# LIONS-EPFL/LEAF

Measured on NVIDIA B200. Metric: leaf_candidates_scored_per_sec, higher is better.
Workload: dtype bf16

## Files before the change

include/leaf_b200.h:

```cpp
#ifndef LEAF_B200_H_
#define LEAF_B200_H_

#include <stdint.h>

#ifdef __cplusplus
extern "C" {
#endif

typedef enum {
  LEAF_OK = 0,
  LEAF_ERR_INVALID = -1,
  LEAF_ERR_CUDA = -2,
  LEAF_ERR_STATE = -3,
  LEAF_ERR_UNSUPPORTED = -4
} leaf_status_t;

typedef struct leaf_engine* leaf_handle_t;

enum { LEAF_ACT_GELU_ERF = 0, LEAF_ACT_QUICK_GELU = 1 };
enum { LEAF_OBJ_L2 = 0, LEAF_OBJ_NEGL2 = 1, LEAF_OBJ_SIM = 2, LEAF_OBJ_DISSIM = 3 };
enum { LEAF_CTX = 77, LEAF_SOT = 49406, LEAF_EOT = 49407, LEAF_VOCAB = 49408, LEAF_N_MERGES = 48894 };
enum { LEAF_MAX_CAPTION_BYTES = 1000, LEAF_MAX_CAPTION_BYTES_LONG = 3560 };

typedef struct {
// ... 33 lines not shown

int leaf_load_bpe(leaf_handle_t h, const uint32_t* merge_pairs_host, int32_t n_merges);

int leaf_bind_weights(leaf_handle_t h, const leaf_weight_ptrs_t* w, void* stream);
int leaf_refresh_weights(leaf_handle_t h, void* stream);

int leaf_reserve(leaf_handle_t h, int32_t max_seqs);

int leaf_expand_tokenize(leaf_handle_t h, const uint8_t* caps, const int32_t* cap_off, int32_t B, int32_t n,
                         const int32_t* pos, const int32_t* chr, const int32_t* sel, const uint8_t* valid,
                         int32_t* tok_out, int32_t* len_out, int32_t* base_out, int32_t* status_out, void* stream);

int leaf_set_tokenizer_mode(leaf_handle_t h, int32_t mode);
int leaf_set_max_caption_bytes(leaf_handle_t h, int32_t bytes);

int leaf_load_words(leaf_handle_t h, const uint8_t* words_blob, const int32_t* words_off, int32_t n_words,
                    const uint8_t* abbrev_blob, const int32_t* abbrev_off, int32_t n_abbrev);
int leaf_constrain_mask(leaf_handle_t h, const uint8_t* caps, const int32_t* cap_off, int32_t B, int32_t n,
                        const int32_t* pos, const int32_t* chr, const int32_t* sel, uint8_t* valid_out,
                        int32_t* count_out, int32_t* status_out, void* stream);

int leaf_encode(leaf_handle_t h, const int32_t* tok, const int32_t* len, const int32_t* base, int32_t N,
                int32_t dedup_rows, int32_t dedup_group, int32_t trim_providers, int32_t normalize, float* feat_out, void* stream);

int leaf_score(leaf_handle_t h, const float* feat, const float* anchor, int32_t B, int32_t n, int32_t objective,
               float* loss_out, int32_t* best_out, float* best_feat_out, void* stream);

int leaf_topk(leaf_handle_t h, const float* score_a, const float* score_b, int32_t m, int32_t k, int32_t* idx_out,
              float* val_out, void* stream);

int leaf_train_reserve(leaf_handle_t h, int32_t max_seqs);
int leaf_forward_train(leaf_handle_t h, const int32_t* tok, const int32_t* len, int32_t N, float* feat_out,
                       int32_t rows_hint, int32_t max_len_hint, int64_t* generation_out, void* stream);
int leaf_backward(leaf_handle_t h, int64_t generation, const float* dfeat, int32_t dfeat_rows, const leaf_weight_ptrs_t* grads,
                  void* stream);

typedef void (*leaf_backward_hook_t)(int32_t layer, void* user);
int leaf_set_backward_hook(leaf_handle_t h, leaf_backward_hook_t fn, void* user);
int leaf_set_sm_budget(leaf_handle_t h, int32_t n_sms);

int leaf_adamw(leaf_handle_t h, float* params, const float* grads, float* exp_avg, float* exp_avg_sq, int64_t n,
               int64_t n_nodecay, float lr, float beta1, float beta2, float eps, float weight_decay, int32_t step,
               float grad_scale, void* stream);
int leaf_sumsq(leaf_handle_t h, const float* g, int64_t n, float* out, void* stream);
int leaf_scale(leaf_handle_t h, float* g, int64_t n, float s, void* stream);

int leaf_gemm_bf16(leaf_handle_t h, const void* A, const void* Bt, const float* bias, void* C,
                   int32_t M, int32_t N, int32_t K, int32_t epilogue, int32_t act, const int32_t* m_dev,
                   void* stream);
int leaf_gemm_bf16_mn(leaf_handle_t h, const void* A, const void* B, const float* bias, void* C, int32_t M, int32_t N,
                      int32_t K, int32_t epilogue, int32_t a_mn, void* stream);
int leaf_test_layernorm(leaf_handle_t h, const float* x, int32_t rows, const float* gamma, const float* beta, void* y,
                        void* stream);
int leaf_test_attention(leaf_handle_t h, const void* qkv, const int32_t* meta, int32_t N, void* out, void* stream);
int leaf_test_attention_bwd(leaf_handle_t h, const void* qkv, const void* o, const float* dout, const int32_t* meta, int32_t N,
                            int32_t T, void* dqkv, void* stream);
int leaf_set_prune_last(leaf_handle_t h, int32_t on);
int64_t leaf_launch_count(leaf_handle_t h, int32_t reset);
int64_t leaf_last_rows(leaf_handle_t h);
int leaf_set_timing(leaf_handle_t h, int32_t on);
double leaf_timing_ms(leaf_handle_t h, int32_t which, int32_t* launches);

#ifdef __cplusplus
}
#endif
#endif
```

leaf_b200/_native.py:

```python
import ctypes
import os

HERE = os.path.dirname(os.path.abspath(__file__))
LIB_PATH = os.environ.get("LEAF_B200_LIB") or os.path.join(HERE, "lib", "libleaf_b200.so")

c_int, c_void_p, c_float, c_i64 = ctypes.c_int32, ctypes.c_void_p, ctypes.c_float, ctypes.c_int64


class LeafCfg(ctypes.Structure):
    _fields_ = [("width", c_int), ("layers", c_int), ("heads", c_int), ("embed_dim", c_int), ("activation", c_int),
                ("ln_eps", c_float)]


class LeafLayerPtrs(ctypes.Structure):
    _fields_ = [(k, c_void_p) for k in (
        "ln1_w", "ln1_b", "in_proj_w", "in_proj_b", "q_w", "k_w", "v_w", "q_b", "k_b", "v_b", "out_w", "out_b",
        "ln2_w", "ln2_b", "fc1_w", "fc1_b", "fc2_w", "fc2_b")]


class LeafWeightPtrs(ctypes.Structure):
    _fields_ = [("token_embedding", c_void_p), ("positional_embedding", c_void_p), ("lnf_w", c_void_p),
                ("lnf_b", c_void_p), ("text_projection", c_void_p), ("projection_is_ew", c_int),
                ("layers", ctypes.POINTER(LeafLayerPtrs))]


SIGNATURES = {
    "leaf_create": (c_int, [ctypes.POINTER(LeafCfg), ctypes.POINTER(c_void_p)]),
    "leaf_destroy": (c_int, [c_void_p]),
    "leaf_last_error": (ctypes.c_char_p, []),
    "leaf_version": (ctypes.c_char_p, []),
    "leaf_load_bpe": (c_int, [c_void_p, c_void_p, c_int]),
    "leaf_bind_weights": (c_int, [c_void_p, ctypes.POINTER(LeafWeightPtrs), c_void_p]),
    "leaf_refresh_weights": (c_int, [c_void_p, c_void_p]),
    "leaf_reserve": (c_int, [c_void_p, c_int]),
    "leaf_expand_tokenize": (c_int, [c_void_p, c_void_p, c_void_p, c_int, c_int, c_void_p, c_void_p, c_void_p, c_void_p,
                                     c_void_p, c_void_p, c_void_p, c_void_p, c_void_p]),
    "leaf_set_tokenizer_mode": (c_int, [c_void_p, c_int]),
    "leaf_set_max_caption_bytes": (c_int, [c_void_p, c_int]),
    "leaf_load_words": (c_int, [c_void_p, c_void_p, c_void_p, c_int, c_void_p, c_void_p, c_int]),
    "leaf_constrain_mask": (c_int, [c_void_p, c_void_p, c_void_p, c_int, c_int, c_void_p, c_void_p, c_void_p, c_void_p, c_void_p,
                                    c_void_p, c_void_p]),
    "leaf_encode": (c_int, [c_void_p, c_void_p, c_void_p, c_void_p, c_int, c_int, c_int, c_int, c_int, c_void_p, c_void_p]),
    "leaf_score": (c_int, [c_void_p, c_void_p, c_void_p, c_int, c_int, c_int, c_void_p, c_void_p, c_void_p, c_void_p]),
    "leaf_topk": (c_int, [c_void_p, c_void_p, c_void_p, c_int, c_int, c_void_p, c_void_p, c_void_p]),
    "leaf_train_reserve": (c_int, [c_void_p, c_int]),
    "leaf_forward_train": (c_int, [c_void_p, c_void_p, c_void_p, c_int, c_void_p, c_int, c_int, ctypes.POINTER(c_i64), c_void_p]),
    "leaf_backward": (c_int, [c_void_p, c_i64, c_void_p, c_int, ctypes.POINTER(LeafWeightPtrs), c_void_p]),
    "leaf_set_backward_hook": (c_int, [c_void_p, c_void_p, c_void_p]),
    "leaf_set_sm_budget": (c_int, [c_void_p, c_int]),
    "leaf_adamw": (c_int, [c_void_p, c_void_p, c_void_p, c_void_p, c_void_p, c_i64, c_i64, ctypes.c_float, ctypes.c_float,
                           ctypes.c_float, ctypes.c_float, ctypes.c_float, c_int, ctypes.c_float, c_void_p]),
    "leaf_sumsq": (c_int, [c_void_p, c_void_p, c_i64, c_void_p, c_void_p]),
    "leaf_scale": (c_int, [c_void_p, c_void_p, c_i64, ctypes.c_float, c_void_p]),
    "leaf_gemm_bf16": (c_int, [c_void_p, c_void_p, c_void_p, c_void_p, c_void_p, c_int, c_int, c_int, c_int, c_int,
                               c_void_p, c_void_p]),
    "leaf_gemm_bf16_mn": (c_int, [c_void_p, c_void_p, c_void_p, c_void_p, c_void_p, c_int, c_int, c_int, c_int, c_int, c_void_p]),
    "leaf_test_layernorm": (c_int, [c_void_p, c_void_p, c_int, c_void_p, c_void_p, c_void_p, c_void_p]),
    "leaf_test_attention": (c_int, [c_void_p, c_void_p, c_void_p, c_int, c_void_p, c_void_p]),
    "leaf_test_attention_bwd": (c_int, [c_void_p, c_void_p, c_void_p, c_void_p, c_void_p, c_int, c_int, c_void_p, c_void_p]),
    "leaf_set_prune_last": (c_int, [c_void_p, c_int]),
    "leaf_launch_count": (c_i64, [c_void_p, c_int]),
    "leaf_last_rows": (c_i64, [c_void_p]),
    "leaf_set_timing": (c_int, [c_void_p, c_int]),
    "leaf_timing_ms": (ctypes.c_double, [c_void_p, c_int, ctypes.POINTER(c_int)]),
}

BACKWARD_HOOK = ctypes.CFUNCTYPE(None, c_int, c_void_p)

_lib = None


class LeafError(RuntimeError):
    pass


def lib():
    global _lib
    if _lib is None:
        if not os.path.exists(LIB_PATH):
            raise LeafError(f"{LIB_PATH} is missing: build it with `python -m leaf_b200.build` "
                            "(leaf_b200 has no CPU or PyTorch fallback)")
        L = ctypes.CDLL(LIB_PATH)
        for name, (res, args) in SIGNATURES.items():
            fn = getattr(L, name)
            fn.restype = res
            fn.argtypes = args
        _lib = L
    return _lib


def check(rc: int):
    if rc != 0:
        raise LeafError(f"leaf_b200 error {rc}: {lib().leaf_last_error().decode('utf-8', 'replace')}")
```

leaf_b200/csrc/engine.cu:

```cuda
#include <cuda.h>
#include <cuda_bf16.h>
#include <cuda_runtime.h>
#include <stdarg.h>
#include <stdint.h>
#include <stdio.h>
#include <stdlib.h>
#include <string.h>

#include <map>
#include <string>
#include <tuple>
#include <vector>

#include "../../include/leaf_b200.h"
#include "gemm2_sm100.cuh"
#include "gemm_sm100.cuh"
#include "k1_tables_host.h"
#include "constrain_kernel.cuh"
#include "k1_tokenize.cuh"
#include "tower_kernels.cuh"
#include "attention2.cuh"
#include "train_kernels.cuh"

using namespace leaf;
// ... 468 lines not shown
  CK(cudaGetLastError());
  return LEAF_OK;
}

template <typename... KArgs, typename... Args>
static cudaError_t launch_pdl(const leaf_engine* e, void (*kernel)(KArgs...), dim3 grid, dim3 block, cudaStream_t st, Args... args) {
  cudaLaunchConfig_t cfg{};
  cfg.gridDim = grid;
  cfg.blockDim = block;
  cfg.stream = st;
  cudaLaunchAttribute attr[1];
  attr[0].id = cudaLaunchAttributeProgrammaticStreamSerialization;
  attr[0].val.programmaticStreamSerializationAllowed = 1;
  cfg.attrs = attr;
  cfg.numAttrs = e->pdl ? 1 : 0;
  return cudaLaunchKernelEx(&cfg, kernel, static_cast<KArgs>(args)...);
}

static int launch_layernorm(leaf_engine* e, const float* x, const int* rows_dev, int rows_max, const int* gather,
                            const float* g, const float* b, __nv_bfloat16* y, cudaStream_t st,
                            const __nv_bfloat16* delta = nullptr, __nv_bfloat16* y_lo = nullptr) {
  const int W = e->cfg.width;
  const int vpl = W / 128;
  TimedSpan span(e, 1, st);
  long warps = rows_max;
  int blocks = static_cast<int>((warps + 7) / 8);
  const int cap = e->sm_count * 8;
  if (blocks > cap) blocks = cap;
  if (blocks < 1) blocks = 1;
#define LN_CASE(V) case V: CK(launch_pdl(e, layernorm_bf16_kernel<V>, dim3(blocks), dim3(256), st, x, rows_dev, rows_max, gather, W, g, b, e->cfg.ln_eps, y, delta, y_lo)); break;
  switch (vpl) {
    LN_CASE(1) LN_CASE(2) LN_CASE(3) LN_CASE(4) LN_CASE(5) LN_CASE(6) LN_CASE(7) LN_CASE(8)
    LN_CASE(9) LN_CASE(10) LN_CASE(11) LN_CASE(12) LN_CASE(13) LN_CASE(14) LN_CASE(15) LN_CASE(16)
    default: return fail(LEAF_ERR_INVALID, "unsupported width %d", W);
  }
#undef LN_CASE
  e->launches++;
  CK(cudaGetLastError());
  return LEAF_OK;
}

static int launch_attention(leaf_engine* e, const __nv_bfloat16* qkv, const int4* meta, int N, __nv_bfloat16* out, int last_only,
                            cudaStream_t st, long rows_cap_hint = 0) {
  if (rows_cap_hint <= 0) rows_cap_hint = static_cast<long>(N) * LEAF_CTX;
  const int H = e->cfg.heads, W = e->cfg.width;
  if (e->att_impl == 2 && static_cast<unsigned long long>(rows_cap_hint) * 3ull * W < (1ull << 32)) {
    const long ctas = (static_cast<long>(N) * H + AT2_WARPS - 1) / AT2_WARPS;
    const int grid2 = static_cast<int>(ctas < 2L * e->sm_count ? ctas : 2L * e->sm_count);
    attention2_kernel<<<grid2, AT2_WARPS * 32, AT2_SMEM_BYTES, st>>>(qkv, meta, N, H, W, out, last_only);
    e->launches++;
    CK(cudaGetLastError());
    return LEAF_OK;
  }
  const int grid = (N * H + ATT_WARPS - 1) / ATT_WARPS;
  CK(launch_pdl(e, attention_kernel, dim3(grid), dim3(ATT_WARPS * 32), st, qkv, meta, N, H, W, out, last_only));
  e->launches++;
  CK(cudaGetLastError());
  return LEAF_OK;
}

extern "C" int leaf_encode(leaf_handle_t e, const int32_t* tok, const int32_t* len, const int32_t* base, int32_t N,
                           int32_t dedup_rows, int32_t dedup_group, int32_t trim_providers, int32_t normalize, float* feat_out,
                           void* stream) {
  if (!e || !tok || !len || !feat_out) return fail(LEAF_ERR_INVALID, "null argument");
  if (!e->bound) return fail(LEAF_ERR_STATE, "weights not bound");
  if (N <= 0) return fail(LEAF_ERR_INVALID, "N=%d", N);
  if (N > e->max_seqs) return fail(LEAF_ERR_STATE, "workspace reserved for %d rows, need %d (leaf_reserve)", e->max_seqs, N);
  cudaStream_t st = static_cast<cudaStream_t>(stream);
  const int W = e->cfg.width, E = e->cfg.embed_dim;
  const int rows_max = static_cast<int>(static_cast<long>(N) * LEAF_CTX);
  int rc;
  const int* dup = nullptr;
  {
  TimedSpan span(e, 3, st);
  if (dedup_group > 1 && dedup_rows > 0) {
    if (dedup_rows > N || dedup_rows % dedup_group != 0) return fail(LEAF_ERR_INVALID, "dedup_rows=%d dedup_group=%d N=%d", dedup_rows, dedup_group, N);
    dedup_kernel<<<(N + 7) / 8, 256, 0, st>>>(tok, len, dedup_rows, dedup_group, N, e->dup_of);
    e->launches++;
    dup = e->dup_of;
  }
  const bool trim = trim_providers && base && dedup_rows > 0 && dedup_rows < N;
  if (trim) CK(cudaMemsetAsync(e->need, 0, static_cast<size_t>(N) * 4, st));
  prefix_kernel<<<(N + 7) / 8, 256, 0, st>>>(tok, len, base, dup, N, e->pfx, e->own_len, trim ? e->need : nullptr);
  if (trim) {
    trim_providers_kernel<<<(N - dedup_rows + 255) / 256, 256, 0, st>>>(base, e->need, dedup_rows, N, e->own_len);
    e->launches++;
  }
  scan_lengths_kernel<<<1, 1024, 0, st>>>(e->own_len, N, e->cu, e->total_rows);
  meta_kernel<<<(N + 255) / 256, 256, 0, st>>>(e->cu, e->pfx, base, dup, N, e->meta, e->eos_row, e->first_of);
  embed_kernel<<<N, 256, 0, st>>>(tok, e->meta, N, W, e->wp.token_embedding, e->wp.positional_embedding, e->x);
  e->launches += 4;
  }
  CK(cudaGetLastError());
  for (int l = 0; l < e->cfg.layers; ++l) {
    const leaf_layer_ptrs_t& p = e->layer_ptrs[l];
    const LayerW& w = e->lw[l];
    if ((rc = launch_layernorm(e, e->x, e->total_rows, rows_max, nullptr, p.ln1_w, p.ln1_b, e->h, st))) return rc;
    if ((rc = launch_gemm(e, e->h, e->rows_cap, w.qkv_w, w.qkv_b, e->big, 3 * W, rows_max, 3 * W, W, EPI_BF16, 0, e->total_rows, st))) return rc;
    const bool last = e->prune_last && l == e->cfg.layers - 1;
    const __nv_bfloat16* dl = e->dlt;
    {
      TimedSpan span(e, 2, st);
      if ((rc = launch_attention(e, e->big, e->meta, N, e->h, last ? 1 : 0, st))) return rc;
    }
    if (last) {
      {
        TimedSpan span(e, 3, st);
// ... 20 lines not shown
  if (normalize) {
    l2_normalize_kernel<<<(N + 7) / 8, 256, 0, st>>>(feat_out, N, E);
    e->launches++;
  }
  CK(cudaGetLastError());
  return LEAF_OK;
}

extern "C" int leaf_score(leaf_handle_t e, const float* feat, const float* anchor, int32_t B, int32_t n, int32_t objective,
                          float* loss_out, int32_t* best_out, float* best_feat_out, void* stream) {
  if (!e || !feat || !anchor || !best_out) return fail(LEAF_ERR_INVALID, "null argument");
  if (B <= 0 || n <= 0 || objective < 0 || objective > 3) return fail(LEAF_ERR_INVALID, "B=%d n=%d objective=%d", B, n, objective);
  if (e->cfg.embed_dim % 4 != 0) return fail(LEAF_ERR_INVALID, "embed_dim");
  if (static_cast<size_t>(n) * 4 > 48 * 1024) return fail(LEAF_ERR_INVALID, "n=%d too large", n);
  score_argmax_kernel<<<B, 256, static_cast<size_t>(n) * 4, static_cast<cudaStream_t>(stream)>>>(
      feat, anchor, n, e->cfg.embed_dim, objective, loss_out, best_out, best_feat_out);
  e->launches++;
  CK(cudaGetLastError());
  return LEAF_OK;
}

extern "C" int leaf_topk(leaf_handle_t e, const float* score_a, const float* score_b, int32_t m, int32_t k, int32_t* idx_out,
                         float* val_out, void* stream) {
  if (!e || !score_a || !idx_out) return fail(LEAF_ERR_INVALID, "null argument");
  if (m <= 0 || k <= 0 || k > m) return fail(LEAF_ERR_INVALID, "top-k of m=%d, k=%d", m, k);
  const size_t smem = static_cast<size_t>(m) * 4;
  if (smem > 200 * 1024) return fail(LEAF_ERR_INVALID, "m=%d too large (max %d)", m, 200 * 1024 / 4);
  topk_kernel<<<1, 1024, smem, static_cast<cudaStream_t>(stream)>>>(score_a, score_b, m, k, idx_out, val_out);
  e->launches++;
  CK(cudaGetLastError());
  return LEAF_OK;
}

extern "C" int leaf_gemm_bf16(leaf_handle_t e, const void* A, const void* Bt, const float* bias, void* C, int32_t M, int32_t N,
                              int32_t K, int32_t epilogue, int32_t act, const int32_t* m_dev, void* stream) {
  if (!e || !A || !Bt || !C) return fail(LEAF_ERR_INVALID, "null argument");
  return launch_gemm(e, static_cast<const __nv_bfloat16*>(A), M, static_cast<const __nv_bfloat16*>(Bt), bias, C, N, M, N, K,
                     epilogue, act, m_dev, static_cast<cudaStream_t>(stream));
}

extern "C" int leaf_gemm_bf16_mn(leaf_handle_t e, const void* A, const void* B, const float* bias, void* C, int32_t M, int32_t N,
                                 int32_t K, int32_t epilogue, int32_t a_mn, void* stream) {
  if (!e || !A || !B || !C) return fail(LEAF_ERR_INVALID, "null argument");
  return launch_gemm(e, static_cast<const __nv_bfloat16*>(A), a_mn ? K : M, static_cast<const __nv_bfloat16*>(B), bias, C, N, M, N, K,
                     epilogue, 0, nullptr, static_cast<cudaStream_t>(stream), nullptr, GEMM_B_MN | (a_mn ? GEMM_A_MN : 0));
}

extern "C" int leaf_test_layernorm(leaf_handle_t e, const float* x, int32_t rows, const float* gamma, const float* beta, void* y,
                                   void* stream) {
  if (!e || !x || !gamma || !beta || !y || rows <= 0) return fail(LEAF_ERR_INVALID, "bad argument");
  return launch_layernorm(e, x, nullptr, rows, nullptr, gamma, beta, static_cast<__nv_bfloat16*>(y), static_cast<cudaStream_t>(stream));
}

extern "C" int leaf_test_attention(leaf_handle_t e, const void* qkv, const int32_t* meta, int32_t N, void* out, void* stream) {
  if (!e || !qkv || !meta || !out || N <= 0) return fail(LEAF_ERR_INVALID, "bad argument");
  return launch_attention(e, static_cast<const __nv_bfloat16*>(qkv), reinterpret_cast<const int4*>(meta), N,
                          static_cast<__nv_bfloat16*>(out), 0, static_cast<cudaStream_t>(stream));
}

extern "C" int leaf_test_attention_bwd(leaf_handle_t e, const void* qkv, const void* o, const float* dout, const int32_t* meta,
                                       int32_t N, int32_t T, void* dqkv, void* stream) {
  if (!e || !qkv || !o || !dout || !meta || !dqkv || N <= 0 || T <= 0 || T > LEAF_CTX) return fail(LEAF_ERR_INVALID, "bad argument");
  attention_bwd_kernel<<<dim3(N, e->cfg.heads), ATTB_WARPS * 32, attb_smem_bytes(T), static_cast<cudaStream_t>(stream)>>>(
      static_cast<const __nv_bfloat16*>(qkv), static_cast<const __nv_bfloat16*>(o), dout, reinterpret_cast<const int4*>(meta),
      e->cfg.width, T, static_cast<__nv_bfloat16*>(dqkv));
  e->launches++;
  CK(cudaGetLastError());
  return LEAF_OK;
}

extern "C" int leaf_set_prune_last(leaf_handle_t e, int32_t on) {
  if (!e) return fail(LEAF_ERR_INVALID, "null handle");
  e->prune_last = on != 0;
  return LEAF_OK;
}

extern "C" int64_t leaf_launch_count(leaf_handle_t e, int32_t reset) {
  if (!e) return 0;
  const int64_t v = e->launches;
  if (reset) e->launches = 0;
  return v;
}

extern "C" int64_t leaf_last_rows(leaf_handle_t e) {
  if (!e || !e->total_rows) return 0;
  int v = 0;
  if (cudaMemcpy(&v, e->total_rows, 4, cudaMemcpyDeviceToHost) != cudaSuccess) return -1;
  return v;
}

extern "C" double leaf_timing_ms(leaf_handle_t e, int32_t which, int32_t* launches);
extern "C" int leaf_set_timing(leaf_handle_t e, int32_t on) {
  if (!e) return fail(LEAF_ERR_INVALID, "null handle");
  e->timing = on != 0;
  if (e->timing) {
    int32_t dummy;
    leaf_timing_ms(e, 0, &dummy);
    for (int i = 0; i < 10; ++i) { e->span_ms[i] = 0; e->span_n[i] = 0; }
  }
  return LEAF_OK;
}

extern "C" double leaf_timing_ms(leaf_handle_t e, int32_t which, int32_t* launches) {
  if (!e || which < 0 || which > 9) return 0.0;
  if (!e->spans.empty()) {
    for (auto& sp : e->spans) {
      cudaEventSynchronize(sp.b);
      float ms = 0.f;
      if (cudaEventElapsedTime(&ms, sp.a, sp.b) == cudaSuccess) {
        e->span_ms[sp.cat] += ms; e->span_n[sp.cat]++;
// ... 344 lines not shown
```

leaf_b200/csrc/tower_kernels.cuh:

```cuda
#pragma once
#include <cuda_bf16.h>
#include <cuda_runtime.h>
#include <stdint.h>

#include "gemm_sm100.cuh"

namespace leaf {

__device__ __forceinline__ float warp_sum(float v) {
#pragma unroll
  for (int o = 16; o > 0; o >>= 1) v += __shfl_xor_sync(0xffffffffu, v, o);
  return v;
}
__device__ __forceinline__ float warp_max(float v) {
#pragma unroll
  for (int o = 16; o > 0; o >>= 1) v = fmaxf(v, __shfl_xor_sync(0xffffffffu, v, o));
  return v;
}

__global__ void __launch_bounds__(1024) scan_lengths_kernel(const int* __restrict__ len, int N, int* __restrict__ cu,
                                                            int* __restrict__ total_rows, int* __restrict__ max_len = nullptr) {
  __shared__ int warp_tot[32];
  __shared__ int carry;
  __shared__ int vmax_s;
// ... 170 lines not shown
      pk.x = *reinterpret_cast<uint32_t*>(&lo);
      pk.y = *reinterpret_cast<uint32_t*>(&hi);
      out[lane + 32 * i] = pk;
      if (y_lo) {
        const float2 l = __bfloat1622float2(lo), h = __bfloat1622float2(hi);
        __nv_bfloat162 lo2 = __floats2bfloat162_rn((v[i].x - mean) * rstd * g.x + b.x - l.x, (v[i].y - mean) * rstd * g.y + b.y - l.y);
        __nv_bfloat162 hi2 = __floats2bfloat162_rn((v[i].z - mean) * rstd * g.z + b.z - h.x, (v[i].w - mean) * rstd * g.w + b.w - h.y);
        uint2 pk2;
        pk2.x = *reinterpret_cast<uint32_t*>(&lo2);
        pk2.y = *reinterpret_cast<uint32_t*>(&hi2);
        reinterpret_cast<uint2*>(y_lo + static_cast<size_t>(r) * W)[lane + 32 * i] = pk2;
      }
    }
  }
}

constexpr int ATT_WARPS = 4;

__device__ __forceinline__ void mma_bf16_16816(float* c, const uint32_t* a, uint32_t b0, uint32_t b1) {
  asm volatile(
      "mma.sync.aligned.m16n8k16.row.col.f32.bf16.bf16.f32 {%0,%1,%2,%3}, {%4,%5,%6,%7}, {%8,%9}, {%0,%1,%2,%3};"
      : "+f"(c[0]), "+f"(c[1]), "+f"(c[2]), "+f"(c[3])
      : "r"(a[0]), "r"(a[1]), "r"(a[2]), "r"(a[3]), "r"(b0), "r"(b1));
}
__device__ __forceinline__ uint32_t movmatrix_trans(uint32_t x) {
  uint32_t y;
  asm volatile("movmatrix.sync.aligned.m8n8.trans.b16 %0, %1;" : "=r"(y) : "r"(x));
  return y;
}
__device__ __forceinline__ uint32_t pack_bf16x2(float lo, float hi) {
  __nv_bfloat162 t = __floats2bfloat162_rn(lo, hi);
  return *reinterpret_cast<uint32_t*>(&t);
}
__device__ __forceinline__ float att_ex2(float x) {
  float y;
  asm("ex2.approx.ftz.f32 %0, %1;" : "=f"(y) : "f"(x));
  return y;
}

struct U8 { uint32_t r[8]; };
__device__ __forceinline__ U8 ldg256(const void* p) {
  U8 v;
  asm volatile("ld.global.nc.v8.b32 {%0,%1,%2,%3,%4,%5,%6,%7}, [%8];"
               : "=r"(v.r[0]), "=r"(v.r[1]), "=r"(v.r[2]), "=r"(v.r[3]), "=r"(v.r[4]), "=r"(v.r[5]), "=r"(v.r[6]), "=r"(v.r[7])
               : "l"(p));
  return v;
}
__device__ __forceinline__ void stg256(void* p, const U8& v) {
  asm volatile("st.global.v8.b32 [%0], {%1,%2,%3,%4,%5,%6,%7,%8};" ::"l"(p), "r"(v.r[0]), "r"(v.r[1]), "r"(v.r[2]), "r"(v.r[3]),
               "r"(v.r[4]), "r"(v.r[5]), "r"(v.r[6]), "r"(v.r[7])
               : "memory");
}

template <int NKT, int DEPTH>
__device__ __forceinline__ void attention_tile(const __nv_bfloat16* __restrict__ kbase, const __nv_bfloat16* __restrict__ vbase,
                                                  size_t ld, const U8& qa, const U8& qb, int pos0, int pos1, int t, int p,
                                                  int own_row, int base_row, int g, int c, float (&o)[8][4], float& inv0, float& inv1) {
  const float sl2 = 0.125f * 1.4426950408889634f;
  constexpr int NS = 2 * NKT;
  U8 ring[DEPTH][2];
  auto issue = [&](int si) {
    const int kt = si < NKT ? si : si - NKT;
    const __nv_bfloat16* src = si < NKT ? kbase : vbase;
#pragma unroll
    for (int h = 0; h < 2; ++h) {
      const int j = min(kt * 16 + h * 8 + g, t - 1);
      ring[si % DEPTH][h] = ldg256(src + static_cast<size_t>(j < p ? base_row + j : own_row + (j - p)) * ld);
    }
  };
#pragma unroll
  for (int si = 0; si < DEPTH && si < NS; ++si) issue(si);
  float s[NKT][2][4];
#pragma unroll
  for (int kt = 0; kt < NKT; ++kt) {
#pragma unroll
    for (int nt = 0; nt < 2; ++nt) {
      s[kt][nt][0] = s[kt][nt][1] = s[kt][nt][2] = s[kt][nt][3] = 0.f;
#pragma unroll
      for (int j = 0; j < 4; ++j) {
        const uint32_t a[4] = {qa.r[2 * j], qb.r[2 * j], qa.r[2 * j + 1], qb.r[2 * j + 1]};
        mma_bf16_16816(s[kt][nt], a, ring[kt % DEPTH][nt].r[2 * j], ring[kt % DEPTH][nt].r[2 * j + 1]);
      }
    }
    if (kt + DEPTH < NS) issue(kt + DEPTH);
  }
  float mx0 = -INFINITY, mx1 = -INFINITY;
#pragma unroll
  for (int kt = 0; kt < NKT; ++kt)
#pragma unroll
    for (int nt = 0; nt < 2; ++nt)
#pragma unroll
      for (int e = 0; e < 2; ++e) {
        const int j = kt * 16 + nt * 8 + 2 * c + e;
        if (j > pos0) s[kt][nt][e] = -INFINITY;
        if (j > pos1) s[kt][nt][2 + e] = -INFINITY;
        mx0 = fmaxf(mx0, s[kt][nt][e]);
        mx1 = fmaxf(mx1, s[kt][nt][2 + e]);
      }
  mx0 = fmaxf(mx0, __shfl_xor_sync(0xffffffffu, mx0, 1));
  mx0 = fmaxf(mx0, __shfl_xor_sync(0xffffffffu, mx0, 2));
  mx1 = fmaxf(mx1, __shfl_xor_sync(0xffffffffu, mx1, 1));
  mx1 = fmaxf(mx1, __shfl_xor_sync(0xffffffffu, mx1, 2));
  const float nm0 = -mx0 * sl2, nm1 = -mx1 * sl2;
  float l0 = 0.f, l1 = 0.f;
  uint32_t pf[NKT][4];
#pragma unroll
  for (int kt = 0; kt < NKT; ++kt)
#pragma unroll
    for (int nt = 0; nt < 2; ++nt) {
      const float p00 = att_ex2(fmaf(s[kt][nt][0], sl2, nm0)), p01 = att_ex2(fmaf(s[kt][nt][1], sl2, nm0));
      const float p10 = att_ex2(fmaf(s[kt][nt][2], sl2, nm1)), p11 = att_ex2(fmaf(s[kt][nt][3], sl2, nm1));
      l0 += p00 + p01;
      l1 += p10 + p11;
      pf[kt][2 * nt] = pack_bf16x2(p00, p01);
      pf[kt][2 * nt + 1] = pack_bf16x2(p10, p11);
    }
  l0 += __shfl_xor_sync(0xffffffffu, l0, 1);
  l0 += __shfl_xor_sync(0xffffffffu, l0, 2);
  l1 += __shfl_xor_sync(0xffffffffu, l1, 1);
  l1 += __shfl_xor_sync(0xffffffffu, l1, 2);
  inv0 = 1.f / l0;
  inv1 = 1.f / l1;
#pragma unroll
  for (int i = 0; i < 8; ++i) o[i][0] = o[i][1] = o[i][2] = o[i][3] = 0.f;
#pragma unroll
  for (int kt = 0; kt < NKT; ++kt) {
#pragma unroll
    for (int i = 0; i < 8; ++i)
      mma_bf16_16816(o[i], pf[kt], movmatrix_trans(ring[(NKT + kt) % DEPTH][0].r[i]), movmatrix_trans(ring[(NKT + kt) % DEPTH][1].r[i]));
    if (NKT + kt + DEPTH < NS) issue(NKT + kt + DEPTH);
  }
}

constexpr int ATT_DEPTH = 3;
__global__ void __launch_bounds__(ATT_WARPS * 32, 4) attention_kernel(const __nv_bfloat16* __restrict__ qkv,
                                                                       const int4* __restrict__ meta, int n_seq, int heads,
                                                                       int W, __nv_bfloat16* __restrict__ out,
                                                                       int last_only = 0) {
  pdl_wait();
  pdl_trigger();
  const int pair = blockIdx.x * ATT_WARPS + (threadIdx.x >> 5);
  if (pair >= n_seq * heads) return;
  const int seq = pair / heads, head = pair - seq * heads;
  const int lane = threadIdx.x & 31, g = lane >> 2, c = lane & 3;
  const int4 mt = __ldg(meta + seq);
  const int own_row = mt.x, t = mt.y, p = mt.z, base_row = mt.w;
  const int nq = t - p;
  if (nq <= 0) return;
  const size_t ld = static_cast<size_t>(3) * W;
  const __nv_bfloat16* qbase = qkv + head * 64 + c * 16;
  const __nv_bfloat16* kbase = qbase + W;
  const __nv_bfloat16* vbase = qbase + 2 * W;
  for (int q0 = last_only ? ((nq - 1) & ~15) : 0; q0 < nq; q0 += 16) {
    const int qi0 = min(q0 + g, nq - 1), qi1 = min(q0 + g + 8, nq - 1);
    const U8 qa = ldg256(qbase + static_cast<size_t>(own_row + qi0) * ld);
    const U8 qb = ldg256(qbase + static_cast<size_t>(own_row + qi1) * ld);
    const int pos0 = p + qi0, pos1 = p + qi1;
    const int kmax = min(t - 1, p + q0 + 15);
    float o[8][4];
    float inv0, inv1;
#define ATT_ARGS kbase, vbase, ld, qa, qb, pos0, pos1, t, p, own_row, base_row, g, c, o, inv0, inv1
    switch (kmax >> 4) {
      case 0: attention_tile<1, ATT_DEPTH>(ATT_ARGS); break;
      case 1: attention_tile<2, ATT_DEPTH>(ATT_ARGS); break;
      case 2: attention_tile<3, ATT_DEPTH>(ATT_ARGS); break;
      case 3: attention_tile<4, ATT_DEPTH>(ATT_ARGS); break;
      default: attention_tile<5, ATT_DEPTH>(ATT_ARGS); break;
    }
#undef ATT_ARGS
    U8 w0, w1;
#pragma unroll
    for (int i = 0; i < 8; ++i) {
      w0.r[i] = pack_bf16x2(o[i][0] * inv0, o[i][1] * inv0);
      w1.r[i] = pack_bf16x2(o[i][2] * inv1, o[i][3] * inv1);
    }
    __nv_bfloat16* ob = out + head * 64 + c * 16;
    if (last_only) {
      if (q0 + g == nq - 1) stg256(ob + static_cast<size_t>(seq) * W, w0);
      if (q0 + g + 8 == nq - 1) stg256(ob + static_cast<size_t>(seq) * W, w1);
    } else {
      if (q0 + g < nq) stg256(ob + static_cast<size_t>(own_row + q0 + g) * W, w0);
      if (q0 + g + 8 < nq) stg256(ob + static_cast<size_t>(own_row + q0 + g + 8) * W, w1);
    }
  }
}

__global__ void __launch_bounds__(256) gather_rows_f32_kernel(const float* __restrict__ src, const int* __restrict__ rows, int N,
                                                             int W, float* __restrict__ dst) {
  const int r = (blockIdx.x * blockDim.x + threadIdx.x) >> 5, lane = threadIdx.x & 31;
  if (r >= N) return;
  const float4* in = reinterpret_cast<const float4*>(src + static_cast<size_t>(rows[r]) * W);
  float4* o = reinterpret_cast<float4*>(dst + static_cast<size_t>(r) * W);
  for (int c = lane; c < W / 4; c += 32) o[c] = in[c];
}

__global__ void __launch_bounds__(256) l2_normalize_kernel(float* __restrict__ f, int N, int E) {
  const int r = (blockIdx.x * blockDim.x + threadIdx.x) >> 5, lane = threadIdx.x & 31;
  if (r >= N) return;
  float* row = f + static_cast<size_t>(r) * E;
  float s = 0.f;
  for (int c = lane; c < E; c += 32) s += row[c] * row[c];
  const float inv = 1.f / fmaxf(sqrtf(warp_sum(s)), 1e-12f);
  for (int c = lane; c < E; c += 32) row[c] *= inv;
}

__global__ void __launch_bounds__(256) score_argmax_kernel(const float* __restrict__ feat, const float* __restrict__ anchor,
                                                          int n, int E, int objective, float* __restrict__ loss_out,
                                                          int* __restrict__ best_out, float* __restrict__ best_feat_out) {
  extern __shared__ float sc[];
  __shared__ float red_v[8];
  __shared__ int red_i[8];
  __shared__ int best_s;
  const int b = blockIdx.x;
  const int warp = threadIdx.x >> 5, lane = threadIdx.x & 31, nwarp = blockDim.x >> 5;
  const float4* a4 = reinterpret_cast<const float4*>(anchor + static_cast<size_t>(b) * E);
  for (int j = warp; j < n; j += nwarp) {
    const float4* f4 = reinterpret_cast<const float4*>(feat + (static_cast<size_t>(b) * n + j) * E);
    float s = 0.f;
    for (int c = lane; c < E / 4; c += 32) {
      const float4 f = f4[c], a = __ldg(a4 + c);
      if (objective <= 1) {
        const float dx = f.x - a.x, dy = f.y - a.y, dz = f.z - a.z, dw = f.w - a.w;
        s += (dx * dx + dy * dy) + (dz * dz + dw * dw);
      } else {
        s += (f.x * a.x + f.y * a.y) + (f.z * a.z + f.w * a.w);
      }
    }
    s = warp_sum(s);
    if (objective == 1 || objective == 3) s = -s;
    if (lane == 0) {
      sc[j] = s;
      if (loss_out) loss_out[static_cast<size_t>(b) * n + j] = s;
    }
  }
  __syncthreads();
  float bv = -INFINITY;
// ... 122 lines not shown
```

leaf_b200/engine.py:

```python
from __future__ import annotations

import ctypes
import os

import numpy as np
import torch

from . import _native
from ._native import LeafCfg, LeafLayerPtrs, LeafWeightPtrs, LeafError, check

HERE = os.path.dirname(os.path.abspath(__file__))
MERGES_BIN = os.path.join(HERE, "data", "clip_bpe_merges.bin")

CONTEXT_LENGTH = 77
OBJECTIVES = {"l2": 0, "negl2": 1, "sim": 2, "dissim": 3}
STATUS_ENTITY_DOMAIN, STATUS_NON_ASCII, STATUS_TOO_LONG = 1, 2, 4
MAX_CAPTION_BYTES = 1000
MAX_CAPTION_BYTES_LONG = 3560
MAX_CODE_POINT = 0x24F


def _ptr(t):
    return None if t is None else ctypes.c_void_p(t.data_ptr())

# ... 295 lines not shown
                                       _ptr(best_feat), _stream()))
        return best, best_feat, loss

    TOPK_MAX = 200 * 1024 // 4

    def topk(self, score_a: torch.Tensor, k: int, m: int = None, score_b: torch.Tensor = None):
        score_a = score_a.reshape(-1)
        m = score_a.numel() if m is None else int(m)
        if score_b is not None:
            score_b = score_b.reshape(-1)
        if m > self.TOPK_MAX:
            idxs, vals = [], []
            for lo in range(0, m, self.TOPK_MAX):
                hi = min(m, lo + self.TOPK_MAX)
                i, v = self.topk(score_a[lo:hi], min(k, hi - lo), score_b=None if score_b is None else score_b[lo:hi])
                idxs.append(i + lo)
                vals.append(v)
            idx_all, val_all = torch.cat(idxs), torch.cat(vals).contiguous()
            if val_all.numel() > self.TOPK_MAX:
                raise LeafError(f"top-{k} of {m} scores needs more than two levels")
            pick, val = self.topk(val_all, k)
            return idx_all[pick.long()].contiguous(), val
        idx = torch.empty((k,), dtype=torch.int32, device=self.device)
        val = torch.empty((k,), dtype=torch.float32, device=self.device)
        with torch.cuda.device(self.device):
            check(self._lib.leaf_topk(self._h, _ptr(score_a.contiguous()), _ptr(None if score_b is None else score_b.contiguous()), m, int(k),
                                      _ptr(idx), _ptr(val), _stream()))
        return idx, val

    def gemm(self, A, Bt, bias=None, epilogue=0, act=0, C=None, m_dev=None):
        M, K = A.shape
        N = Bt.shape[0]
        if C is None:
            C = torch.empty((M, N), dtype=torch.bfloat16 if epilogue in (0, 1) else torch.float32, device=A.device)
        with torch.cuda.device(self.device):
            check(self._lib.leaf_gemm_bf16(self._h, _ptr(A), _ptr(Bt), _ptr(bias), _ptr(C), M, N, K, epilogue, act, _ptr(m_dev), _stream()))
        return C

    def gemm_mn(self, A, B, bias=None, epilogue=3, C=None, a_mn=True):
        K, N = B.shape
        M = A.shape[1] if a_mn else A.shape[0]
        if C is None:
            C = torch.zeros((M, N), dtype=torch.bfloat16 if epilogue in (0, 1) else torch.float32, device=A.device)
        with torch.cuda.device(self.device):
            check(self._lib.leaf_gemm_bf16_mn(self._h, _ptr(A), _ptr(B), _ptr(bias), _ptr(C), M, N, K, epilogue, 1 if a_mn else 0,
                                              _stream()))
        return C

    def test_layernorm(self, x, gamma, beta):
        y = torch.empty(x.shape, dtype=torch.bfloat16, device=x.device)
        check(self._lib.leaf_test_layernorm(self._h, _ptr(x), x.shape[0], _ptr(gamma), _ptr(beta), _ptr(y), _stream()))
        return y

    def test_attention(self, qkv, meta, out=None):
        if out is None:
            out = torch.zeros((qkv.shape[0], self.width), dtype=torch.bfloat16, device=qkv.device)
        check(self._lib.leaf_test_attention(self._h, _ptr(qkv), _ptr(meta), meta.shape[0], _ptr(out), _stream()))
        return out

    def test_attention_bwd(self, qkv, o, dout, meta, T):
        dqkv = torch.zeros_like(qkv)
        check(self._lib.leaf_test_attention_bwd(self._h, _ptr(qkv), _ptr(o), _ptr(dout), _ptr(meta), meta.shape[0], int(T),
                                                _ptr(dqkv), _stream()))
        return dqkv

    def set_prune_last(self, on: bool):
        check(self._lib.leaf_set_prune_last(self._h, 1 if on else 0))

    def launch_count(self, reset=False) -> int:
        return int(self._lib.leaf_launch_count(self._h, 1 if reset else 0))

    def set_timing(self, on: bool):
        check(self._lib.leaf_set_timing(self._h, 1 if on else 0))

    def gemm_time_ms(self):
        return self.class_time_ms(0)

    def class_time_ms(self, which: int):
        n = ctypes.c_int32(0)
        ms = self._lib.leaf_timing_ms(self._h, int(which), ctypes.byref(n))
        return float(ms), int(n.value)

    def last_rows(self) -> int:
        return int(self._lib.leaf_last_rows(self._h))


def _text_config(module):
    cfg = getattr(module, "config", None)
    cfg = getattr(cfg, "text_config", None) or cfg
    act = getattr(cfg, "hidden_act", None)
    if cfg is None or act is None or not hasattr(cfg, "num_attention_heads"):
        return None
    if act not in ("quick_gelu", "gelu"):
        raise LeafError(f"unsupported text-tower activation {act!r} (the engine has nn.GELU and QuickGELU)")
    return int(cfg.num_attention_heads), act == "quick_gelu", float(getattr(cfg, "layer_norm_eps", 1e-5))


def _open_clip_config(module):
    text = getattr(module, "text", module)
    blocks = getattr(getattr(text, "transformer", None), "resblocks", None)
    if blocks is None or len(blocks) == 0:
        raise LeafError("cannot find transformer.resblocks in the module (open_clip naming expected)")
    blk = blocks[0]
    heads = getattr(getattr(blk, "attn", None), "num_heads", None)
    if heads is None:
        raise LeafError("cannot infer the number of attention heads of the tower")
    acts = {type(m).__name__ for m in blk.modules()}
    quick = bool(acts & {"QuickGELU", "QuickGELUActivation"})
    if not quick and not acts & {"GELU", "GELUActivation"}:
        raise LeafError(f"cannot tell the MLP activation of the tower (module classes: {sorted(acts)})")
# ... 28 lines not shown
```

Measured before the change: 77040.

## Process two attention heads per warp with precomputed key row offsets

The forward attention kernel now gives each warp a pair of heads instead of one. It computes the K/V row indices once, streams both heads' K and V tiles through a single prefetch ring, and loads the second head's Q during the first head's PV step. Row addresses are formed with inline mad.wide, and the causal mask is applied only to the last two key tiles. The grid is halved and the minimum-blocks launch bound drops from 4 to 3, which raises the register budget per thread but lowers occupancy. The test entry point also gains a last_only parameter.

```diff
diff --git a/include/leaf_b200.h b/include/leaf_b200.h
--- a/include/leaf_b200.h
+++ b/include/leaf_b200.h
@@ -109,7 +109,8 @@
                       int32_t K, int32_t epilogue, int32_t a_mn, void* stream);
 int leaf_test_layernorm(leaf_handle_t h, const float* x, int32_t rows, const float* gamma, const float* beta, void* y,
                         void* stream);
-int leaf_test_attention(leaf_handle_t h, const void* qkv, const int32_t* meta, int32_t N, void* out, void* stream);
+int leaf_test_attention(leaf_handle_t h, const void* qkv, const int32_t* meta, int32_t N, void* out, int32_t last_only,
+                        void* stream);
 int leaf_test_attention_bwd(leaf_handle_t h, const void* qkv, const void* o, const float* dout, const int32_t* meta, int32_t N,
                             int32_t T, void* dqkv, void* stream);
 int leaf_set_prune_last(leaf_handle_t h, int32_t on);
diff --git a/leaf_b200/_native.py b/leaf_b200/_native.py
--- a/leaf_b200/_native.py
+++ b/leaf_b200/_native.py
@@ -56,7 +56,7 @@
                                c_void_p, c_void_p]),
     "leaf_gemm_bf16_mn": (c_int, [c_void_p, c_void_p, c_void_p, c_void_p, c_void_p, c_int, c_int, c_int, c_int, c_int, c_void_p]),
     "leaf_test_layernorm": (c_int, [c_void_p, c_void_p, c_int, c_void_p, c_void_p, c_void_p, c_void_p]),
-    "leaf_test_attention": (c_int, [c_void_p, c_void_p, c_void_p, c_int, c_void_p, c_void_p]),
+    "leaf_test_attention": (c_int, [c_void_p, c_void_p, c_void_p, c_int, c_void_p, c_int, c_void_p]),
     "leaf_test_attention_bwd": (c_int, [c_void_p, c_void_p, c_void_p, c_void_p, c_void_p, c_int, c_int, c_void_p, c_void_p]),
     "leaf_set_prune_last": (c_int, [c_void_p, c_int]),
     "leaf_launch_count": (c_i64, [c_void_p, c_int]),
diff --git a/leaf_b200/csrc/engine.cu b/leaf_b200/csrc/engine.cu
--- a/leaf_b200/csrc/engine.cu
+++ b/leaf_b200/csrc/engine.cu
@@ -544,7 +544,7 @@
     CK(cudaGetLastError());
     return LEAF_OK;
   }
-  const int grid = (N * H + ATT_WARPS - 1) / ATT_WARPS;
+  const int grid = (N * (H / 2) + ATT_WARPS - 1) / ATT_WARPS;
   CK(launch_pdl(e, attention_kernel, dim3(grid), dim3(ATT_WARPS * 32), st, qkv, meta, N, H, W, out, last_only));
   e->launches++;
   CK(cudaGetLastError());
@@ -671,10 +671,11 @@
   return launch_layernorm(e, x, nullptr, rows, nullptr, gamma, beta, static_cast<__nv_bfloat16*>(y), static_cast<cudaStream_t>(stream));
 }
 
-extern "C" int leaf_test_attention(leaf_handle_t e, const void* qkv, const int32_t* meta, int32_t N, void* out, void* stream) {
+extern "C" int leaf_test_attention(leaf_handle_t e, const void* qkv, const int32_t* meta, int32_t N, void* out, int32_t last_only,
+                                   void* stream) {
   if (!e || !qkv || !meta || !out || N <= 0) return fail(LEAF_ERR_INVALID, "bad argument");
   return launch_attention(e, static_cast<const __nv_bfloat16*>(qkv), reinterpret_cast<const int4*>(meta), N,
-                          static_cast<__nv_bfloat16*>(out), 0, static_cast<cudaStream_t>(stream));
+                          static_cast<__nv_bfloat16*>(out), last_only ? 1 : 0, static_cast<cudaStream_t>(stream));
 }
 
 extern "C" int leaf_test_attention_bwd(leaf_handle_t e, const void* qkv, const void* o, const float* dout, const int32_t* meta,
diff --git a/leaf_b200/csrc/tower_kernels.cuh b/leaf_b200/csrc/tower_kernels.cuh
--- a/leaf_b200/csrc/tower_kernels.cuh
+++ b/leaf_b200/csrc/tower_kernels.cuh
@@ -246,96 +246,133 @@
                : "memory");
 }
 
+template <typename T>
+__device__ __forceinline__ T* att_row_addr(T* base, int row, int ld_bytes) {
+  T* a;
+  asm volatile("mad.wide.s32 %0, %1, %2, %3;" : "=l"(a) : "r"(row), "r"(ld_bytes), "l"(base));
+  return a;
+}
+
 template <int NKT, int DEPTH>
-__device__ __forceinline__ void attention_tile(const __nv_bfloat16* __restrict__ kbase, const __nv_bfloat16* __restrict__ vbase,
-                                                  size_t ld, const U8& qa, const U8& qb, int pos0, int pos1, int t, int p,
-                                                  int own_row, int base_row, int g, int c, float (&o)[8][4], float& inv0, float& inv1) {
+__device__ __forceinline__ void attention_pair_tile(const __nv_bfloat16* __restrict__ qbase, __nv_bfloat16* __restrict__ obase,
+                                                    int W, const U8& qa, const U8& qb, int qr0, int qr1, int or0, int or1,
+                                                    int pos0, int pos1, int t, int p, int own_row, int base_row, int g) {
+  const int ld_bytes = 6 * W;
+  const __nv_bfloat16* kbase = qbase + W;
   const float sl2 = 0.125f * 1.4426950408889634f;
-  constexpr int NS = 2 * NKT;
+  constexpr int NS = 4 * NKT;
+  int krow[NKT][2];
+#pragma unroll
+  for (int kt = 0; kt < NKT; ++kt)
+#pragma unroll
+    for (int h = 0; h < 2; ++h) {
+      const int j = kt == NKT - 1 ? min(kt * 16 + h * 8 + g, t - 1) : kt * 16 + h * 8 + g;
+      krow[kt][h] = j < p ? base_row + j : own_row + (j - p);
+    }
   U8 ring[DEPTH][2];
   auto issue = [&](int si) {
-    const int kt = si < NKT ? si : si - NKT;
-    const __nv_bfloat16* src = si < NKT ? kbase : vbase;
-#pragma unroll
-    for (int h = 0; h < 2; ++h) {
-      const int j = min(kt * 16 + h * 8 + g, t - 1);
-      ring[si % DEPTH][h] = ldg256(src + static_cast<size_t>(j < p ? base_row + j : own_row + (j - p)) * ld);
-    }
+    const int hd = si / (2 * NKT), r = si % (2 * NKT);
+    const int kt = r < NKT ? r : r - NKT;
+    const __nv_bfloat16* src = kbase + (r < NKT ? 0 : W) + hd * 64;
+#pragma unroll
+    for (int h = 0; h < 2; ++h) ring[si % DEPTH][h] = ldg256(att_row_addr(src, krow[kt][h], ld_bytes));
   };
 #pragma unroll
   for (int si = 0; si < DEPTH && si < NS; ++si) issue(si);
-  float s[NKT][2][4];
-#pragma unroll
-  for (int kt = 0; kt < NKT; ++kt) {
-#pragma unroll
-    for (int nt = 0; nt < 2; ++nt) {
-      s[kt][nt][0] = s[kt][nt][1] = s[kt][nt][2] = s[kt][nt][3] = 0.f;
-#pragma unroll
-      for (int j = 0; j < 4; ++j) {
-        const uint32_t a[4] = {qa.r[2 * j], qb.r[2 * j], qa.r[2 * j + 1], qb.r[2 * j + 1]};
-        mma_bf16_16816(s[kt][nt], a, ring[kt % DEPTH][nt].r[2 * j], ring[kt % DEPTH][nt].r[2 * j + 1]);
-      }
-    }
-    if (kt + DEPTH < NS) issue(kt + DEPTH);
-  }
-  float mx0 = -INFINITY, mx1 = -INFINITY;
-#pragma unroll
-  for (int kt = 0; kt < NKT; ++kt)
-#pragma unroll
-    for (int nt = 0; nt < 2; ++nt)
-#pragma unroll
-      for (int e = 0; e < 2; ++e) {
-        const int j = kt * 16 + nt * 8 + 2 * c + e;
-        if (j > pos0) s[kt][nt][e] = -INFINITY;
-        if (j > pos1) s[kt][nt][2 + e] = -INFINITY;
-        mx0 = fmaxf(mx0, s[kt][nt][e]);
-        mx1 = fmaxf(mx1, s[kt][nt][2 + e]);
-      }
-  mx0 = fmaxf(mx0, __shfl_xor_sync(0xffffffffu, mx0, 1));
-  mx0 = fmaxf(mx0, __shfl_xor_sync(0xffffffffu, mx0, 2));
-  mx1 = fmaxf(mx1, __shfl_xor_sync(0xffffffffu, mx1, 1));
-  mx1 = fmaxf(mx1, __shfl_xor_sync(0xffffffffu, mx1, 2));
-  const float nm0 = -mx0 * sl2, nm1 = -mx1 * sl2;
-  float l0 = 0.f, l1 = 0.f;
-  uint32_t pf[NKT][4];
-#pragma unroll
-  for (int kt = 0; kt < NKT; ++kt)
-#pragma unroll
-    for (int nt = 0; nt < 2; ++nt) {
-      const float p00 = att_ex2(fmaf(s[kt][nt][0], sl2, nm0)), p01 = att_ex2(fmaf(s[kt][nt][1], sl2, nm0));
-      const float p10 = att_ex2(fmaf(s[kt][nt][2], sl2, nm1)), p11 = att_ex2(fmaf(s[kt][nt][3], sl2, nm1));
-      l0 += p00 + p01;
-      l1 += p10 + p11;
-      pf[kt][2 * nt] = pack_bf16x2(p00, p01);
-      pf[kt][2 * nt + 1] = pack_bf16x2(p10, p11);
-    }
-  l0 += __shfl_xor_sync(0xffffffffu, l0, 1);
-  l0 += __shfl_xor_sync(0xffffffffu, l0, 2);
-  l1 += __shfl_xor_sync(0xffffffffu, l1, 1);
-  l1 += __shfl_xor_sync(0xffffffffu, l1, 2);
-  inv0 = 1.f / l0;
-  inv1 = 1.f / l1;
-#pragma unroll
-  for (int i = 0; i < 8; ++i) o[i][0] = o[i][1] = o[i][2] = o[i][3] = 0.f;
-#pragma unroll
-  for (int kt = 0; kt < NKT; ++kt) {
-#pragma unroll
-    for (int i = 0; i < 8; ++i)
-      mma_bf16_16816(o[i], pf[kt], movmatrix_trans(ring[(NKT + kt) % DEPTH][0].r[i]), movmatrix_trans(ring[(NKT + kt) % DEPTH][1].r[i]));
-    if (NKT + kt + DEPTH < NS) issue(NKT + kt + DEPTH);
+  U8 qbA = qa, qbB = qb;
+#pragma unroll
+  for (int hd = 0; hd < 2; ++hd) {
+    const int s0 = hd * 2 * NKT;
+    float s[NKT][2][4];
+#pragma unroll
+    for (int kt = 0; kt < NKT; ++kt) {
+#pragma unroll
+      for (int nt = 0; nt < 2; ++nt) {
+        s[kt][nt][0] = s[kt][nt][1] = s[kt][nt][2] = s[kt][nt][3] = 0.f;
+#pragma unroll
+        for (int j = 0; j < 4; ++j) {
+          const uint32_t a[4] = {qbA.r[2 * j], qbB.r[2 * j], qbA.r[2 * j + 1], qbB.r[2 * j + 1]};
+          mma_bf16_16816(s[kt][nt], a, ring[(s0 + kt) % DEPTH][nt].r[2 * j], ring[(s0 + kt) % DEPTH][nt].r[2 * j + 1]);
+        }
+      }
+      if (s0 + kt + DEPTH < NS) issue(s0 + kt + DEPTH);
+    }
+    const int c = threadIdx.x & 3;
+    float mx0 = -INFINITY, mx1 = -INFINITY;
+#pragma unroll
+    for (int kt = 0; kt < NKT; ++kt)
+#pragma unroll
+      for (int nt = 0; nt < 2; ++nt)
+#pragma unroll
+        for (int e = 0; e < 2; ++e) {
+          if (kt >= NKT - 2) {
+            const int j = kt * 16 + nt * 8 + 2 * c + e;
+            if (j > pos0) s[kt][nt][e] = -INFINITY;
+            if (j > pos1) s[kt][nt][2 + e] = -INFINITY;
+          }
+          mx0 = fmaxf(mx0, s[kt][nt][e]);
+          mx1 = fmaxf(mx1, s[kt][nt][2 + e]);
+        }
+    mx0 = fmaxf(mx0, __shfl_xor_sync(0xffffffffu, mx0, 1));
+    mx0 = fmaxf(mx0, __shfl_xor_sync(0xffffffffu, mx0, 2));
+    mx1 = fmaxf(mx1, __shfl_xor_sync(0xffffffffu, mx1, 1));
+    mx1 = fmaxf(mx1, __shfl_xor_sync(0xffffffffu, mx1, 2));
+    const float nm0 = -mx0 * sl2, nm1 = -mx1 * sl2;
+    float l0 = 0.f, l1 = 0.f;
+    uint32_t pf[NKT][4];
+#pragma unroll
+    for (int kt = 0; kt < NKT; ++kt)
+#pragma unroll
+      for (int nt = 0; nt < 2; ++nt) {
+        const float p00 = att_ex2(fmaf(s[kt][nt][0], sl2, nm0)), p01 = att_ex2(fmaf(s[kt][nt][1], sl2, nm0));
+        const float p10 = att_ex2(fmaf(s[kt][nt][2], sl2, nm1)), p11 = att_ex2(fmaf(s[kt][nt][3], sl2, nm1));
+        l0 += p00 + p01;
+        l1 += p10 + p11;
+        pf[kt][2 * nt] = pack_bf16x2(p00, p01);
+        pf[kt][2 * nt + 1] = pack_bf16x2(p10, p11);
+      }
+    l0 += __shfl_xor_sync(0xffffffffu, l0, 1);
+    l0 += __shfl_xor_sync(0xffffffffu, l0, 2);
+    l1 += __shfl_xor_sync(0xffffffffu, l1, 1);
+    l1 += __shfl_xor_sync(0xffffffffu, l1, 2);
+    const float inv0 = 1.f / l0, inv1 = 1.f / l1;
+    if (hd == 0) {
+      qbA = ldg256(att_row_addr(qbase + 64, qr0, ld_bytes));
+      qbB = ldg256(att_row_addr(qbase + 64, qr1, ld_bytes));
+    }
+    float o[8][4];
+#pragma unroll
+    for (int i = 0; i < 8; ++i) o[i][0] = o[i][1] = o[i][2] = o[i][3] = 0.f;
+#pragma unroll
+    for (int kt = 0; kt < NKT; ++kt) {
+      const int sv = s0 + NKT + kt;
+#pragma unroll
+      for (int i = 0; i < 8; ++i)
+        mma_bf16_16816(o[i], pf[kt], movmatrix_trans(ring[sv % DEPTH][0].r[i]), movmatrix_trans(ring[sv % DEPTH][1].r[i]));
+      if (sv + DEPTH < NS) issue(sv + DEPTH);
+    }
+    U8 w0, w1;
+#pragma unroll
+    for (int i = 0; i < 8; ++i) {
+      w0.r[i] = pack_bf16x2(o[i][0] * inv0, o[i][1] * inv0);
+      w1.r[i] = pack_bf16x2(o[i][2] * inv1, o[i][3] * inv1);
+    }
+    if (or0 >= 0) stg256(att_row_addr(obase + hd * 64, or0, 2 * W), w0);
+    if (or1 >= 0) stg256(att_row_addr(obase + hd * 64, or1, 2 * W), w1);
   }
 }
 
 constexpr int ATT_DEPTH = 3;
-__global__ void __launch_bounds__(ATT_WARPS * 32, 4) attention_kernel(const __nv_bfloat16* __restrict__ qkv,
+__global__ void __launch_bounds__(ATT_WARPS * 32, 3) attention_kernel(const __nv_bfloat16* __restrict__ qkv,
                                                                        const int4* __restrict__ meta, int n_seq, int heads,
                                                                        int W, __nv_bfloat16* __restrict__ out,
                                                                        int last_only = 0) {
   pdl_wait();
   pdl_trigger();
-  const int pair = blockIdx.x * ATT_WARPS + (threadIdx.x >> 5);
-  if (pair >= n_seq * heads) return;
-  const int seq = pair / heads, head = pair - seq * heads;
+  const int pairs = heads >> 1;
+  const int item = blockIdx.x * ATT_WARPS + (threadIdx.x >> 5);
+  if (item >= n_seq * pairs) return;
+  const int seq = item / pairs, head = 2 * (item - seq * pairs);
   const int lane = threadIdx.x & 31, g = lane >> 2, c = lane & 3;
   const int4 mt = __ldg(meta + seq);
   const int own_row = mt.x, t = mt.y, p = mt.z, base_row = mt.w;
@@ -343,39 +380,30 @@
   if (nq <= 0) return;
   const size_t ld = static_cast<size_t>(3) * W;
   const __nv_bfloat16* qbase = qkv + head * 64 + c * 16;
-  const __nv_bfloat16* kbase = qbase + W;
-  const __nv_bfloat16* vbase = qbase + 2 * W;
+  __nv_bfloat16* ob = out + head * 64 + c * 16;
   for (int q0 = last_only ? ((nq - 1) & ~15) : 0; q0 < nq; q0 += 16) {
     const int qi0 = min(q0 + g, nq - 1), qi1 = min(q0 + g + 8, nq - 1);
     const U8 qa = ldg256(qbase + static_cast<size_t>(own_row + qi0) * ld);
     const U8 qb = ldg256(qbase + static_cast<size_t>(own_row + qi1) * ld);
     const int pos0 = p + qi0, pos1 = p + qi1;
     const int kmax = min(t - 1, p + q0 + 15);
-    float o[8][4];
-    float inv0, inv1;
-#define ATT_ARGS kbase, vbase, ld, qa, qb, pos0, pos1, t, p, own_row, base_row, g, c, o, inv0, inv1
+    int or0 = -1, or1 = -1;
+    if (last_only) {
+      if (q0 + g == nq - 1) or0 = seq;
+      if (q0 + g + 8 == nq - 1) or1 = seq;
+    } else {
+      if (q0 + g < nq) or0 = own_row + q0 + g;
+      if (q0 + g + 8 < nq) or1 = own_row + q0 + g + 8;
+    }
+#define ATT_ARGS qbase, ob, W, qa, qb, own_row + qi0, own_row + qi1, or0, or1, pos0, pos1, t, p, own_row, base_row, g
     switch (kmax >> 4) {
-      case 0: attention_tile<1, ATT_DEPTH>(ATT_ARGS); break;
-      case 1: attention_tile<2, ATT_DEPTH>(ATT_ARGS); break;
-      case 2: attention_tile<3, ATT_DEPTH>(ATT_ARGS); break;
-      case 3: attention_tile<4, ATT_DEPTH>(ATT_ARGS); break;
-      default: attention_tile<5, ATT_DEPTH>(ATT_ARGS); break;
+      case 0: attention_pair_tile<1, ATT_DEPTH>(ATT_ARGS); break;
+      case 1: attention_pair_tile<2, ATT_DEPTH>(ATT_ARGS); break;
+      case 2: attention_pair_tile<3, ATT_DEPTH>(ATT_ARGS); break;
+      case 3: attention_pair_tile<4, ATT_DEPTH>(ATT_ARGS); break;
+      default: attention_pair_tile<5, ATT_DEPTH>(ATT_ARGS); break;
     }
 #undef ATT_ARGS
-    U8 w0, w1;
-#pragma unroll
-    for (int i = 0; i < 8; ++i) {
-      w0.r[i] = pack_bf16x2(o[i][0] * inv0, o[i][1] * inv0);
-      w1.r[i] = pack_bf16x2(o[i][2] * inv1, o[i][3] * inv1);
-    }
-    __nv_bfloat16* ob = out + head * 64 + c * 16;
-    if (last_only) {
-      if (q0 + g == nq - 1) stg256(ob + static_cast<size_t>(seq) * W, w0);
-      if (q0 + g + 8 == nq - 1) stg256(ob + static_cast<size_t>(seq) * W, w1);
-    } else {
-      if (q0 + g < nq) stg256(ob + static_cast<size_t>(own_row + q0 + g) * W, w0);
-      if (q0 + g + 8 < nq) stg256(ob + static_cast<size_t>(own_row + q0 + g + 8) * W, w1);
-    }
   }
 }
 
diff --git a/leaf_b200/engine.py b/leaf_b200/engine.py
--- a/leaf_b200/engine.py
+++ b/leaf_b200/engine.py
@@ -371,10 +371,12 @@
         check(self._lib.leaf_test_layernorm(self._h, _ptr(x), x.shape[0], _ptr(gamma), _ptr(beta), _ptr(y), _stream()))
         return y
 
-    def test_attention(self, qkv, meta, out=None):
+    def test_attention(self, qkv, meta, out=None, last_only=False):
         if out is None:
-            out = torch.zeros((qkv.shape[0], self.width), dtype=torch.bfloat16, device=qkv.device)
-        check(self._lib.leaf_test_attention(self._h, _ptr(qkv), _ptr(meta), meta.shape[0], _ptr(out), _stream()))
+            rows = meta.shape[0] if last_only else qkv.shape[0]
+            out = torch.zeros((rows, self.width), dtype=torch.bfloat16, device=qkv.device)
+        check(self._lib.leaf_test_attention(self._h, _ptr(qkv), _ptr(meta), meta.shape[0], _ptr(out), 1 if last_only else 0,
+                                            _stream()))
         return out
 
     def test_attention_bwd(self, qkv, o, dout, meta, T):
```

Result: no change. 77410, median of 6 (+0.5%).
